# Unrepentant-Atheist/AC-3-ACM-Codec

Measured on AMD Instinct MI355X. Metric: AC-3 5.1@48kHz frames/sec/GPU (decode+encode); achieved HBM GB/s vs peak, higher is better.
Workload: dtype f32+i32

## Files before the change

### ac-3-acm-codec_amd/csrc/decode_mx.hip

```cpp
#include <stdlib.h>
#include "mant2.h"
#include "xform_core.h"
#include "ac3mi_internal.h"

namespace ac3mi {

constexpr int MX_PLANE = 256 + 16;
constexpr int MX_WAVE = 6 * EX_GROUP * 8;
constexpr int MX_RING = 6 * MX_PLANE * 4;
constexpr int MX_TILE = 3072;
static_assert(MX_RING + M2_LDS_WAVE <= MX_WAVE && MX_TILE + 256 * 6 * 2 <= MX_WAVE && 48 * 8 * 8 <= MX_TILE, "region layout");

struct MantxParams {
    MantParams m;
    const uint8_t *blksw;
    float *delay;
    const int32_t *slot;
    int delay_stride;
    float *pcm;
    int16_t *pcm16;
    int8_t wslot[6];
    const float2 *tw_long, *tw_short;
    const float *window;
    float bias;
};

struct MantxLDS {
    uint4 dsc[M2_NDESC];
    float qtab[760];
    float2 tw[2][128];
    float win[256];
    uint8_t cplbnd[6][20];
    uint32_t ready[6];
    alignas(16) uint8_t wave[6][MX_WAVE];
};

#ifndef MANTX_LB
#define MANTX_LB 3
#endif
#ifdef MX_STAMPS
__device__ unsigned long long g_mx_cycles[6][8];
#define MX_T0() unsigned long long mx_t = __builtin_readcyclecounter()
#define MX_LAP(id) do { const unsigned long long t_ = __builtin_readcyclecounter(); if (lane == 0) atomicAdd(&g_mx_cycles[blk][id], t_ - mx_t); mx_t = t_; } while (0)
#else
#define MX_T0() do { } while (0)
#define MX_LAP(id) do { } while (0)
#endif
template <bool S16>
__global__ __launch_bounds__(384, MANTX_LB) void mantx_kernel(const MantxParams Q)
{
    const MantParams &P = Q.m;
    __shared__ MantxLDS L;
    extern __shared__ uint32_t frw[];
    const int tid = threadIdx.x, lane = tid & 63;
    const int blk = __builtin_amdgcn_readfirstlane(tid >> 6);
    MX_T0();
    unsigned fidx;
    {
        const unsigned n = gridDim.x, q = n >> 3, r = n & 7u, x = blockIdx.x & 7u, i = blockIdx.x >> 3;
        fidx = (x < r ? x * (q + 1) : r * (q + 1) + (x - r) * q) + i;
    }
    const size_t unit = (size_t)fidx * 6 + blk;
    const uint4 *dq = reinterpret_cast<const uint4 *>(P.desc + unit);
    const uint4 w0v = dq[0], w1v = dq[1], w2v = dq[2], w3v = dq[3], w4v = dq[4];
    const uint32_t fposv = P.frame_pos[fidx];
    const int nw = (P.frame_bytes + 3) >> 2;
    {
        const uint32_t *s32 = reinterpret_cast<const uint32_t *>(P.frames + (size_t)fidx * P.frame_stride);
        for (int i = tid; i < nw + 6; i += 384) {
            uint32_t v = 0;
            if (i < nw) {
                v = s32[i];
                const int rem = P.frame_bytes - 4 * i;
                if (rem < 4) v &= (1u << (8 * rem)) - 1u;
                v = __builtin_bswap32(v);
            }
            frw[i] = v;
        }
        if (tid < M2_NDESC) L.dsc[tid] = mant_desc2((uint32_t)tid);
        for (int i = tid; i < 760; i += 384) L.qtab[i] = P.tab->qtab[i];
        if (tid < 128) L.tw[0][tid] = Q.tw_long[tid];
        else if (tid < 256) L.tw[1][tid - 128] = Q.tw_short[tid - 128];
        else L.win[tid - 256] = Q.window[tid - 256];
        if (tid < 128) L.win[128 + tid] = Q.window[128 + tid];
        if (tid < 6) L.ready[tid] = 0u;
    }
    uint8_t *const region = L.wave[blk];
    float *const planes = reinterpret_cast<float *>(region);
    const uint32_t flags = rfl(w0v.z);
    const bool failed = (flags & 1u) != 0u;
    MantBlk B;
    B.nf = P.nfchans; B.lfeon = P.lfeon; B.acmod = P.acmod; B.in_lfe = P.lfeon ? 1 : 0;
    B.chincpl = (int)((flags >> 8) & 31u); B.dithmask = (int)((flags >> 16) & 31u); B.rematflg = (int)((flags >> 24) & 15u);
    const uint64_t rve = (uint64_t)rfl(w2v.x) | ((uint64_t)rfl(w2v.y) << 32), rvb = (uint64_t)rfl(w2v.z) | ((uint64_t)rfl(w2v.w) << 32);
    const uint8_t *rowbase = P.rows + (size_t)fidx * 6 * ROWSET;
    auto fetch = [&](int slot) -> uint2 {
        const uint8_t *er = rowbase + (size_t)((rve >> (8 * slot)) & 7u) * ROWSET + slot * 512;
        const uint8_t *br = rowbase + (size_t)((rvb >> (8 * slot)) & 7u) * ROWSET + slot * 512 + 256;
        if (slot == 5) return lane < 7 ? make_uint2(br[lane], er[lane]) : make_uint2(1u, 0u);
        return make_uint2(reinterpret_cast<const uint32_t *>(br)[lane], reinterpret_cast<const uint32_t *>(er)[lane]);
    };
    const int slot0 = seg_slot(0, B.nf, B.chincpl, B.chincpl ? __builtin_ctz(B.chincpl) : 99);
    uint2 first = make_uint2(0u, 0u);
    if (!failed) first = fetch(slot0);
    __syncthreads();
    MX_LAP(0);

    if (failed) {
        for (int c = 0; c < P.n_in; c++)
            *reinterpret_cast<float4 *>(planes + c * MX_PLANE + 4 * lane) = make_float4(0.f, 0.f, 0.f, 0.f);
    } else {
        {
            const uint32_t a = rfl(w1v.x), b = rfl(w1v.y), c = rfl(w1v.z), d = rfl(w1v.w);
            B.cplstrtmant = (int)(c >> 16); B.cplendmant = (int)(d & 0xffffu);
            B.ends = (uint64_t)((a & 0xffu) | ((a >> 8) & 0xff00u) | ((b & 0xffu) << 16) | ((b << 8) & 0xff000000u)) | ((uint64_t)(c & 0xffu) << 32);
        }
        B.gainv = lane == 0 ? __uint_as_float(w3v.x) : lane == 1 ? __uint_as_float(w3v.y) : lane == 2 ? __uint_as_float(w3v.z)
                : lane == 3 ? __uint_as_float(w3v.w) : lane == 4 ? __uint_as_float(w4v.x) : __uint_as_float(w4v.y);
        if (B.chincpl && lane < 18) {
            const uint32_t below = rfl(w0v.w) & ((1u << lane) - 1u);
            L.cplbnd[blk][lane] = (uint8_t)(lane - __popc(below));
        }
        const uint32_t fpos = rfl(fposv);
        const bool lfsr_live = fpos != 0xffffffffu;
        const uint32_t i0 = lfsr_live ? (fpos + rfl(w0v.y)) % 65535u : 0u;
        const float *cc = P.cplco + unit * 90;
        mant_block2<MX_PLANE, true>(B, fetch, first, [&](int c, int bnd) { return cc[c * 18 + bnd]; }, L.cplbnd[blk], L.dsc, region + MX_RING, frw,
                              (uint32_t)nw + 2u, L.qtab, reinterpret_cast<const int16_t *>(P.lfsr_seq) + 1 + i0, lfsr_live, planes, rfl(w0v.x), lane);
    }
    __builtin_amdgcn_fence(__ATOMIC_RELEASE, "wavefront");
    __builtin_amdgcn_wave_barrier();
    __builtin_amdgcn_fence(__ATOMIC_ACQUIRE, "wavefront");

    MX_LAP(1);
    const int l8 = lane & 7, grp = lane >> 3;
    const bool own = grp < P.n_in;
    const int o = own ? grp : 0;
    const int fb = o - B.in_lfe;
    const bool sw = fb >= 0 && Q.blksw[unit * P.nfchans + fb] != 0;
    const size_t sidx = Q.slot ? (size_t)Q.slot[fidx] : (size_t)fidx;
    float *const dptr = Q.delay + sidx * Q.delay_stride + (size_t)o * 128;
    float2 dl[8];
    if (blk == 0) {
#pragma unroll
        for (int j = 0; j < 8; j++) {
            const int i = ((j & 1) ? 15 - l8 : l8) + 16 * (j >> 1);
            dl[j] = *reinterpret_cast<const float2 *>(dptr + 2 * i);
        }
    }
    FirstTail ft;
#pragma unroll
    for (int j = 0; j < 8; j++) ft.f0[j] = ft.f1[j] = ft.t0[j] = ft.t1[j] = 0.f;
    {
        const float *plane = planes + o * MX_PLANE;
        float xa[16], xb[16];
        if (!sw) {
            const float2 *p = reinterpret_cast<const float2 *>(plane) + l8;
            float2 v[16];
#pragma unroll
            for (int n = 0; n < 16; n++) v[n] = p[8 * n];
#pragma unroll
            for (int n = 0; n < 16; n++) {
                xa[n] = __builtin_fmaf(1.f, v[n].x, 0.f);
                xb[n] = __builtin_fmaf(1.f, mirror8(v[15 - n].y), 0.f);
            }
        } else {
            const int f = l8 >> 2, n2 = l8 & 3;
            const float *pa = plane + 4 * n2 + f;
            const float *pb = plane + 254 + f - 4 * n2;
#pragma unroll
            for (int n = 0; n < 16; n++) {
                xa[n] = __builtin_fmaf(1.f, pa[16 * n], 0.f);
                xb[n] = __builtin_fmaf(1.f, pb[-16 * n], 0.f);
            }
        }
        __builtin_amdgcn_fence(__ATOMIC_RELEASE, "wavefront");
        __builtin_amdgcn_wave_barrier();
        __builtin_amdgcn_fence(__ATOMIC_ACQUIRE, "wavefront");
        float2 *ex = reinterpret_cast<float2 *>(region) + o * EX_GROUP;
        const float2 *tw = &L.tw[sw ? 1 : 0][l8 * 16];
        cf r[16];
        imdct_first_half(xa, xb, tw, ex, l8, r);
        if (!sw) imdct_long_second_half(r, ft);
        else imdct_short_second_half(r, ft);
    }
    __builtin_amdgcn_fence(__ATOMIC_RELEASE, "wavefront");
    __builtin_amdgcn_wave_barrier();
    if (blk < 5 && lane < 48) {
        float2 *tl = reinterpret_cast<float2 *>(region);
#pragma unroll
        for (int j = 0; j < 8; j++) tl[j * 48 + lane] = make_float2(ft.t0[j], ft.t1[j]);
    }
    MX_LAP(2);
    if (blk == 0) asm volatile("s_waitcnt vmcnt(0)" ::: "memory");
    if (blk < 5) __hip_atomic_store(&L.ready[blk], 1u, __ATOMIC_RELEASE, __HIP_MEMORY_SCOPE_WORKGROUP);
    if (blk > 0) {
        for (int spin = 0; spin < (1 << 20) && __hip_atomic_load(&L.ready[blk - 1], __ATOMIC_ACQUIRE, __HIP_MEMORY_SCOPE_WORKGROUP) == 0u; spin++)
            __builtin_amdgcn_s_sleep(1);
        const float2 *tl = reinterpret_cast<const float2 *>(L.wave[blk - 1]);
        const int ls = lane < 48 ? lane : l8;
#pragma unroll
        for (int j = 0; j < 8; j++) dl[j] = tl[j * 48 + ls];
    }
    if (blk == 5) {
        for (int spin = 0; spin < (1 << 20) && __hip_atomic_load(&L.ready[0], __ATOMIC_ACQUIRE, __HIP_MEMORY_SCOPE_WORKGROUP) == 0u; spin++)
            __builtin_amdgcn_s_sleep(1);
    }
    if (blk == 5 && own) {
#pragma unroll
        for (int j = 0; j < 8; j++) {
            const int i = ((j & 1) ? 15 - l8 : l8) + 16 * (j >> 1);
            *reinterpret_cast<float2 *>(dptr + 2 * i) = make_float2(ft.t0[j], ft.t1[j]);
        }
    }

    MX_LAP(3);
    int16_t *tile = reinterpret_cast<int16_t *>(region + MX_TILE);
    int wsl = 0;
#pragma unroll
    for (int oo = 0; oo < 6; oo++) wsl = oo == o ? Q.wslot[oo] : wsl;
    float *oblk = S16 ? nullptr : Q.pcm + (unit * P.n_in + o) * 256;
#pragma unroll
    for (int j = 0; j < 8; j++) {
        const int i = ((j & 1) ? 15 - l8 : l8) + 16 * (j >> 1);
        const float2 wlo = *reinterpret_cast<const float2 *>(&L.win[2 * i]);
        const float2 whi = *reinterpret_cast<const float2 *>(&L.win[254 - 2 * i]);
        float2 lo, hi;
        window_pair(ft.f0[j], ft.f1[j], dl[j], wlo, whi, Q.bias, lo, hi);
        if (!S16 && own) {
            *reinterpret_cast<float2 *>(oblk + 2 * i) = lo;
            *reinterpret_cast<float2 *>(oblk + 254 - 2 * i) = hi;
        }
        if (S16 && own) {
            const int at = wsl + (int)__umul24((uint32_t)(2 * i), (uint32_t)P.n_in), top = wsl + (int)__umul24(254u, (uint32_t)P.n_in) - (at - wsl);
            tile[at] = to_s16(lo.x);
            tile[at + P.n_in] = to_s16(lo.y);
            tile[top] = to_s16(hi.x);
            tile[top + P.n_in] = to_s16(hi.y);
        }
    }
    if (S16) {
        __builtin_amdgcn_fence(__ATOMIC_RELEASE, "wavefront");
        __builtin_amdgcn_wave_barrier();
        __builtin_amdgcn_fence(__ATOMIC_ACQUIRE, "wavefront");
        const int upb = 32 * P.n_in;
        int16_t *dst = Q.pcm16 + unit * 256 * P.n_in;
#pragma unroll
        for (int it = 0; it < 3; it++) {
            const int u = it * 64 + lane;
            if (u < upb) *reinterpret_cast<uint4 *>(dst + u * 8) = *reinterpret_cast<const uint4 *>(tile + u * 8);
        }
    }
    MX_LAP(4);
}

hipError_t launch_mantx(const DeviceTables &tab, const DecodeLaunch &L, const MantParams &M, hipStream_t stream)
{
    const XformLaunch &X = *L.fuse;
    if (L.frames_per_stream != 1 || X.plan.n_in != X.plan.n_out || M.n_in > 6) return hipErrorInvalidValue;
    MantxParams Q;
    Q.m = M;
    Q.m.coef = nullptr;
    Q.blksw = L.blksw;
    Q.delay = X.delay;
    Q.slot = X.slot;
    Q.delay_stride = X.slot ? X.delay_stride : X.plan.n_out * 128;
    Q.pcm = X.pcm;
    Q.pcm16 = X.pcm16;
    Q.tw_long = tab.tw_long;
    Q.tw_short = tab.tw_short;
    Q.window = tab.window;
    Q.bias = X.bias;
    for (int o = 0; o < 6; o++) Q.wslot[o] = 0;
    static const int lds_pad = getenv("AC3MI_MANTX_LDS_PAD") ? atoi(getenv("AC3MI_MANTX_LDS_PAD")) : 0;
    const size_t dyn = (size_t)(((L.frame_bytes + 3) >> 2) + 6) * 4 + lds_pad;
    if (X.pcm16) {
        int map[6];
        if (s16_channel_map(X.s16_flags, map) != X.plan.n_out || ((uintptr_t)X.pcm16 & 15)) return hipErrorInvalidValue;
        for (int w = 0; w < X.plan.n_out; w++) Q.wslot[map[w]] = (int8_t)w;
        hipLaunchKernelGGL(mantx_kernel<true>, dim3(M.n_frames), dim3(384), dyn, stream, Q);
    } else {
        hipLaunchKernelGGL(mantx_kernel<false>, dim3(M.n_frames), dim3(384), dyn, stream, Q);
    }
    return hipGetLastError();
}

}

#ifdef MX_STAMPS
extern "C" __attribute__((visibility("default"))) int ac3mi_debug_mx_cycles(unsigned long long *out48, int reset)
{
    if (hipMemcpyFromSymbol(out48, HIP_SYMBOL(ac3mi::g_mx_cycles), sizeof(unsigned long long) * 48) != hipSuccess) return -1;
    if (reset) { unsigned long long z[48] = {0}; if (hipMemcpyToSymbol(HIP_SYMBOL(ac3mi::g_mx_cycles), z, sizeof z) != hipSuccess) return -1; }
    return 0;
}
#endif
```

### ac-3-acm-codec_amd/csrc/mant2.h

```cpp
#pragma once
#include "decode_common.h"

namespace ac3mi {

constexpr int M2_RING = 3 * 128;
constexpr int M2_LDS_WAVE = M2_RING + 256;
constexpr int M2_NDESC = 97;
constexpr int LFSR_EXT = 16384;

__host__ __device__ inline uint4 mant_desc2(uint32_t b)
{
    const uint32_t k1 = b >> 5, nbp = b >= 32 ? 0u : b == 1 ? 0u : b;
    const uint32_t inc = k1 == 1 ? 1u << 20 : k1 == 2 ? 1u << 10 : k1 == 3 ? 1u : 0u;
    const uint32_t obits = k1 == 1 ? 5u : k1 ? 7u : 0u, per = k1 == 3 ? 2u : k1 ? 3u : 0u, sh = 30u - 10u * k1;
    const uint32_t recip = k1 == 3 ? 1024u : k1 ? 683u : 0u;
    const uint32_t qbase = k1 == 1 ? 0u : k1 == 2 ? 96u : k1 == 3 ? 480u : nbp == 3 ? 736u : nbp == 4 ? 744u : 0u;
    const uint32_t coded = (k1 || nbp == 3 || nbp == 4) ? 1u : 0u, zero = b == 0 ? 1u : 0u;
    const uint32_t ring = k1 ? 128u * (k1 - 1u) : 0u;
    return make_uint4(inc, nbp | (obits << 8) | (per << 16) | (sh << 24), recip | (qbase << 16), ring | (zero << 16) | (coded << 24));
}

struct MantParams {
    const uint8_t *frames;
    const BlkDesc *desc;
    const uint8_t *rows;
    const float *cplco;
    const uint32_t *frame_pos;
    float *coef;
    const uint16_t *lfsr_seq;
    const DecTables *tab;
    unsigned n_frames;
    int frame_stride, frame_bytes;
    int acmod, lfeon, n_in, nfchans;
};

struct Seg2 {
    uint32_t bit;
    uint32_t phase;
    uint32_t draw;
};

template <int NB>
struct Bins2 {
    uint32_t raw[NB];
    uint32_t rs[NB];
    uint32_t dy[NB], dz[NB], dw[NB];
    uint32_t cd;
};

template <int NB>
__device__ __forceinline__ void seg2_first(uint32_t bytes4, const uint4 *dsc, uint8_t *ring, const uint32_t *frw, uint32_t frw_last,
                                           int mult, Seg2 &S, Bins2<NB> &R, int lane)
{
    uint32_t inc[NB], gl = 0;
#pragma unroll
    for (int j = 0; j < NB; j++) {
        const uint32_t b = (bytes4 >> (8 * j)) & 0xffu;
        const uint4 d = dsc[b];
        inc[j] = d.x; R.dy[j] = d.y; R.dz[j] = d.z; R.dw[j] = d.w;
        gl += d.x;
    }
    const uint32_t gin = wave_incl_scan_u32(gl);
    uint32_t run = gin - gl + S.phase;
    uint32_t nb[NB], nbsum = 0, ndsum = 0, slot[NB];
#pragma unroll
    for (int j = 0; j < NB; j++) {
        const uint32_t x = __builtin_amdgcn_ubfe(run, R.dy[j] >> 24, 10);
        run += inc[j];
        const uint32_t q = (x * (R.dz[j] & 0xffffu)) >> 11;
        const uint32_t mem = x - q * ((R.dy[j] >> 16) & 0xffu);
        const uint32_t ob = mem == 0u ? (R.dy[j] >> 8) & 0xffu : 0u;
        nb[j] = (R.dy[j] & 0xffu) + ob;
        nbsum += nb[j];
        ndsum += ((R.dw[j] >> 16) & 0xffu) * (uint32_t)mult;
        const uint32_t rslot = (R.dw[j] & 0xffffu) + (q & 127u);
        R.rs[j] = rslot | (mem << 16);
        slot[j] = ob != 0u ? rslot : (uint32_t)(M2_RING + 4 * lane);
    }
    const uint32_t bl = nbsum | (ndsum << 16);
    const uint32_t bin_ = wave_incl_scan_u32(bl);
    const uint32_t gtot = wave_last(gin), btot = wave_last(bin_);
    R.cd = S.draw + (bin_ >> 16) - ndsum;
    const uint32_t off = S.bit + (bin_ & 0xffffu) - nbsum;
    uint32_t wi = off >> 5;
    wi = wi < frw_last ? wi : frw_last;
    const uint32_t d0 = frw[wi], d1 = frw[wi + 1], d2 = frw[wi + 2];
    const uint32_t k = off & 31u;
    uint64_t win = ((((uint64_t)d0 << 32) | d1) << k) | (uint64_t)((d2 >> 1) >> (31u - k));
#pragma unroll
    for (int j = 0; j < NB; j++) {
        R.raw[j] = ((uint32_t)(win >> 32) >> 1) >> (31u - nb[j]);
        win <<= nb[j];
        ring[slot[j]] = (uint8_t)R.raw[j];
    }
    S.bit += btot & 0xffffu;
    S.draw += btot >> 16;
    {
        const uint32_t x3 = ((S.phase >> 20) & 1023u) + ((gtot >> 20) & 1023u), x5 = ((S.phase >> 10) & 1023u) + ((gtot >> 10) & 1023u),
                       x11 = (S.phase & 1023u) + (gtot & 1023u);
        const uint32_t q3 = (x3 * 683u) >> 11, q5 = (x5 * 683u) >> 11, q11 = x11 >> 1;
        S.phase = (((q3 & 127u) * 3u + (x3 - 3u * q3)) << 20) | (((q5 & 127u) * 3u + (x5 - 3u * q5)) << 10) | ((q11 & 127u) * 2u + (x11 & 1u));
    }
}

template <int NB>
__device__ __forceinline__ void seg2_values(const Bins2<NB> &R, const uint8_t *ring, const float *qtab, float *q)
{
    uint32_t code[NB];
#pragma unroll
    for (int j = 0; j < NB; j++) code[j] = ring[R.rs[j] & 0xffffu];
#pragma unroll
    for (int j = 0; j < NB; j++) { asm volatile("" : "+v"(code[j])); code[j] &= 0xffu; }
    float tv[NB];
#pragma unroll
    for (int j = 0; j < NB; j++) {
        const uint32_t per = (R.dy[j] >> 16) & 0xffu;
        const uint32_t sel = per ? code[j] * per + (R.rs[j] >> 16) : R.raw[j];
        tv[j] = qtab[(R.dw[j] >> 24) ? (R.dz[j] >> 16) + sel : 0u];
    }
#pragma unroll
    for (int j = 0; j < NB; j++) {
        const uint32_t nbp = R.dy[j] & 0xffu;
        const float pv = (float)(((int32_t)(R.raw[j] << ((32u - nbp) & 31u))) >> 16);
        q[j] = (R.dw[j] >> 24) ? tv[j] : pv;
    }
}

__device__ __forceinline__ float dither2(const int16_t *seq, uint32_t i) { return (float)((3 * (int)seq[i]) >> 2); }

template <int PS = 256, bool PK = false, class Fetch, class Cplco>
__device__ __forceinline__ void mant_block2(const MantBlk &B, Fetch fetch, uint2 first, Cplco cplco_of, const uint8_t *cplbnd, const uint4 *dsc, uint8_t *ring,
                                            const uint32_t *frw, uint32_t frw_last, const float *qtab, const int16_t *seq1, bool lfsr_live,
                                            float *cblk, uint32_t bitpos, int lane)
{
    const int nf = B.nf;
    const int ncpl_dith = __popc(B.chincpl & B.dithmask);
    const int em0 = PK ? (int)((uint32_t)B.ends & 0xffu) : B.endmant[0], em1 = PK ? (int)(((uint32_t)B.ends >> 8) & 0xffu) : B.endmant[1];
    const int remat_end = em0 < em1 ? em0 : em1;
    const bool remat_late = B.acmod == 2 && B.rematflg != 0 && B.chincpl != 0 && remat_end > B.cplstrtmant;
    const int cplfirst = B.chincpl ? __builtin_ctz(B.chincpl) : 99;
    const int nseg = nf + (B.chincpl ? 1 : 0) + (B.lfeon ? 1 : 0);
    Seg2 S;
    S.bit = bitpos;
    S.phase = 0;
    S.draw = 0;
    uint2 nxt = first;
    for (int k = 0; k < nseg; k++) {
        const int slot = seg_slot(k, nf, B.chincpl, cplfirst);
        const uint2 cur = nxt;
        if (k + 1 < nseg) nxt = fetch(seg_slot(k + 1, nf, B.chincpl, cplfirst));
        if (slot == 5) {
            Bins2<1> R;
            seg2_first<1>(lane < 7 ? cur.x & 0xffu : 1u, dsc, ring, frw, frw_last, 0, S, R, lane);
            __builtin_amdgcn_fence(__ATOMIC_RELEASE, "wavefront");
            __builtin_amdgcn_wave_barrier();
            __builtin_amdgcn_fence(__ATOMIC_ACQUIRE, "wavefront");
            float q;
            seg2_values<1>(R, ring, qtab, &q);
            const float lfe_gain = PK ? __builtin_bit_cast(float, __builtin_amdgcn_readlane(__builtin_bit_cast(int, B.gainv), 5)) : B.lfe_gain;
            const float v = q * (sf_of((int)(cur.y & 0xffu)) * lfe_gain);
            const float z = 0.f * (sf_of(0) * lfe_gain);
            if (lane < 8) cblk[lane] = lane < 7 ? v : z;
            if (lane >= 2) *reinterpret_cast<float4 *>(cblk + 4 * lane) = make_float4(z, z, z, z);
            continue;
        }
        int start = 0, end, draws;
        float g = 0.f;
        if (slot < 5) {
            if (PK) {
                end = (int)((uint32_t)(B.ends >> (8 * slot)) & 0xffu);
                g = __builtin_bit_cast(float, __builtin_amdgcn_readlane(__builtin_bit_cast(int, B.gainv), slot));
            } else {
                end = slot == 0 ? B.endmant[0] : slot == 1 ? B.endmant[1] : slot == 2 ? B.endmant[2] : slot == 3 ? B.endmant[3] : B.endmant[4];
                g = slot == 0 ? B.gain[0] : slot == 1 ? B.gain[1] : slot == 2 ? B.gain[2] : slot == 3 ? B.gain[3] : B.gain[4];
            }
            draws = (B.dithmask >> slot) & 1;
        } else {
            start = B.cplstrtmant;
            end = B.cplendmant;
            draws = ncpl_dith;
        }
        uint32_t bytes4;
        {
            int lo = start - 4 * lane, hi = end - 4 * lane;
            lo = lo < 0 ? 0 : lo > 4 ? 4 : lo;
            hi = hi < 0 ? 0 : hi > 4 ? 4 : hi;
            const uint32_t below_hi = (uint32_t)((1ull << (8 * hi)) - 1ull), below_lo = (uint32_t)((1ull << (8 * lo)) - 1ull);
            const uint32_t m = below_hi & ~below_lo;
            bytes4 = (cur.x & m) | (0x01010101u & ~m);
        }
        Bins2<4> R;
        seg2_first<4>(bytes4, dsc, ring, frw, frw_last, draws, S, R, lane);
        __builtin_amdgcn_fence(__ATOMIC_RELEASE, "wavefront");
        __builtin_amdgcn_wave_barrier();
        __builtin_amdgcn_fence(__ATOMIC_ACQUIRE, "wavefront");
        if (slot < 5) {
            float out[4], qv[4];
            seg2_values<4>(R, ring, qtab, qv);
            const bool dith = draws != 0 && lfsr_live;
            const uint32_t z0 = (R.dw[0] >> 16) & 0xffu, z1 = (R.dw[1] >> 16) & 0xffu, z2 = (R.dw[2] >> 16) & 0xffu, z3 = (R.dw[3] >> 16) & 0xffu;
            if (dith && __any((z0 | z1 | z2 | z3) != 0u)) {
                const int16_t *sp = seq1 + R.cd;
                const float d0 = dither2(sp, 0), d1 = dither2(sp, z0), d2 = dither2(sp, z0 + z1), d3 = dither2(sp, z0 + z1 + z2);
                qv[0] = z0 ? d0 : qv[0]; qv[1] = z1 ? d1 : qv[1]; qv[2] = z2 ? d2 : qv[2]; qv[3] = z3 ? d3 : qv[3];
            }
#pragma unroll
            for (int j = 0; j < 4; j++) {
                const int e = (int)((cur.y >> (8 * j)) & 0xffu);
                out[j] = qv[j] * (sf_of(e) * g);
            }
            float *plane = cblk + (slot + B.in_lfe) * PS;
            if (slot == 1 && B.acmod == 2 && B.rematflg != 0 && !remat_late) {
                float4 a4 = *reinterpret_cast<const float4 *>(plane - PS + 4 * lane);
                float a[4] = {a4.x, a4.y, a4.z, a4.w};
#pragma unroll
                for (int j = 0; j < 4; j++) {
                    const int bin = 4 * lane + j;
                    const int band = bin < 25 ? 0 : bin < 37 ? 1 : bin < 61 ? 2 : 3;
                    if (bin >= 13 && (bin < remat_end || (bin == 13 && remat_end <= 13)) && ((B.rematflg >> band) & 1)) {
                        const float x = a[j], v = out[j];
                        a[j] = x + v;
                        out[j] = x - v;
                    }
                }
                *reinterpret_cast<float4 *>(plane - PS + 4 * lane) = make_float4(a[0], a[1], a[2], a[3]);
            }
            if ((B.chincpl >> slot) & 1) {
#pragma unroll
                for (int j = 0; j < 4; j++) {
                    const int bin = 4 * lane + j;
                    if (bin < end || bin < B.cplstrtmant || bin >= B.cplendmant) plane[bin] = bin >= B.cplendmant ? 0.f : out[j];
                }
            } else {
                *reinterpret_cast<float4 *>(plane + 4 * lane) = make_float4(out[0], out[1], out[2], out[3]);
            }
        } else {
            uint32_t cd = R.cd;
            float qv[4];
            seg2_values<4>(R, ring, qtab, qv);
#pragma unroll
            for (int j = 0; j < 4; j++) {
                const int bin = 4 * lane + j;
                const bool in = bin >= start && bin < end;
                const bool zero = ((R.dw[j] >> 16) & 0xffu) != 0u;
                const int e = (int)((cur.y >> (8 * j)) & 0xffu);
                const float m = qv[j] * sf_of(e);
                const int bnd = cplbnd[in ? (bin - start) / 12 : 0];
                uint32_t cdc = cd;
                for (int c = 0; c < nf; c++) {
                    if (!((B.chincpl >> c) & 1)) continue;
                    const float gc = PK ? __builtin_bit_cast(float, __builtin_amdgcn_readlane(__builtin_bit_cast(int, B.gainv), c))
                                        : c == 0 ? B.gain[0] : c == 1 ? B.gain[1] : c == 2 ? B.gain[2] : c == 3 ? B.gain[3] : B.gain[4];
                    const float co = cplco_of(c, bnd) * gc;
                    float v = m * co;
                    if (zero) {
                        v = 0.f;
                        if ((B.dithmask >> c) & 1) { v = (sf_of(e) * co) * (lfsr_live ? dither2(seq1, cdc) : 0.f); cdc++; }
                    }
                    if (in) cblk[(c + B.in_lfe) * PS + bin] = v;
                }
                cd += zero ? (uint32_t)draws : 0u;
            }
        }
    }
    if (remat_late) {
        __builtin_amdgcn_fence(__ATOMIC_RELEASE, "wavefront");
        __builtin_amdgcn_wave_barrier();
        __builtin_amdgcn_fence(__ATOMIC_ACQUIRE, "wavefront");
        volatile float *p0 = cblk + (size_t)B.in_lfe * PS, *p1 = p0 + PS;
        for (int bin = 13 + lane; bin < remat_end; bin += 64) {
            const int band = bin < 25 ? 0 : bin < 37 ? 1 : bin < 61 ? 2 : 3;
            if ((B.rematflg >> band) & 1) {
                const float a = p0[bin], v = p1[bin];
                p0[bin] = a + v;
                p1[bin] = a - v;
            }
        }
    }
}

}
```

### ac-3-acm-codec_amd/csrc/xform_core.h

```cpp
#pragma once
#include <hip/hip_runtime.h>

namespace ac3mi {

struct cf { float re, im; };

__device__ __forceinline__ cf operator+(cf a, cf b) { return {a.re + b.re, a.im + b.im}; }
__device__ __forceinline__ cf operator-(cf a, cf b) { return {a.re - b.re, a.im - b.im}; }
__device__ __forceinline__ cf cmul(cf a, float cr, float ci)
{
    return {__builtin_fmaf(a.re, cr, -(a.im * ci)), __builtin_fmaf(a.re, ci, a.im * cr)};
}
__device__ __forceinline__ cf cmul(cf a, cf c) { return cmul(a, c.re, c.im); }

__device__ constexpr float C32_RE[16] = {
    1.000000000e+00f, 9.951847267e-01f, 9.807852804e-01f, 9.569403357e-01f, 9.238795325e-01f,
    8.819212643e-01f, 8.314696123e-01f, 7.730104534e-01f, 7.071067812e-01f, 6.343932842e-01f,
    5.555702330e-01f, 4.713967368e-01f, 3.826834324e-01f, 2.902846773e-01f, 1.950903220e-01f,
    9.801714033e-02f};
__device__ constexpr float C32_IM[16] = {
    -0.000000000e+00f, -9.801714033e-02f, -1.950903220e-01f, -2.902846773e-01f, -3.826834324e-01f,
    -4.713967368e-01f, -5.555702330e-01f, -6.343932842e-01f, -7.071067812e-01f, -7.730104534e-01f,
    -8.314696123e-01f, -8.819212643e-01f, -9.238795325e-01f, -9.569403357e-01f, -9.807852804e-01f,
    -9.951847267e-01f};

constexpr float K_C1 = 9.238795325e-01f;
constexpr float K_S1 = 3.826834324e-01f;
constexpr float K_R2 = 7.071067812e-01f;

__device__ __forceinline__ void dft4(cf &a, cf &b, cf &c, cf &d)
{
    cf s0 = a + c, s1 = a - c, s2 = b + d, s3 = b - d;
    a = s0 + s2;
    c = s0 - s2;
    b = {s1.re + s3.im, s1.im - s3.re};
    d = {s1.re - s3.im, s1.im + s3.re};
}

__device__ __forceinline__ void dft16(cf (&v)[16])
{
#pragma unroll
    for (int n2 = 0; n2 < 4; n2++) dft4(v[n2], v[4 + n2], v[8 + n2], v[12 + n2]);
    v[5] = cmul(v[5], K_C1, -K_S1);
    v[6] = {(v[6].re + v[6].im) * K_R2, (v[6].im - v[6].re) * K_R2};
    v[7] = cmul(v[7], K_S1, -K_C1);
    v[9] = {(v[9].re + v[9].im) * K_R2, (v[9].im - v[9].re) * K_R2};
    v[10] = {v[10].im, -v[10].re};
    v[11] = {(v[11].im - v[11].re) * K_R2, -(v[11].re + v[11].im) * K_R2};
    v[13] = cmul(v[13], K_S1, -K_C1);
    v[14] = {(v[14].im - v[14].re) * K_R2, -(v[14].re + v[14].im) * K_R2};
    v[15] = cmul(v[15], -K_C1, K_S1);
#pragma unroll
    for (int k1 = 0; k1 < 4; k1++) dft4(v[4 * k1], v[4 * k1 + 1], v[4 * k1 + 2], v[4 * k1 + 3]);
    cf t;
    t = v[1]; v[1] = v[4]; v[4] = t;
    t = v[2]; v[2] = v[8]; v[8] = t;
    t = v[3]; v[3] = v[12]; v[12] = t;
    t = v[6]; v[6] = v[9]; v[9] = t;
    t = v[7]; v[7] = v[13]; v[13] = t;
    t = v[11]; v[11] = v[14]; v[14] = t;
}

__device__ __forceinline__ void dft8(cf &a0, cf &a1, cf &a2, cf &a3, cf &a4, cf &a5, cf &a6, cf &a7)
{
    dft4(a0, a2, a4, a6);
    dft4(a1, a3, a5, a7);
    a3 = {(a3.re + a3.im) * K_R2, (a3.im - a3.re) * K_R2};
    a5 = {a5.im, -a5.re};
    a7 = {(a7.im - a7.re) * K_R2, -(a7.re + a7.im) * K_R2};
    cf x0 = a0 + a1, x4 = a0 - a1, x1 = a2 + a3, x5 = a2 - a3;
    cf x2 = a4 + a5, x6 = a4 - a5, x3 = a6 + a7, x7 = a6 - a7;
    a0 = x0; a1 = x1; a2 = x2; a3 = x3; a4 = x4; a5 = x5; a6 = x6; a7 = x7;
}

__device__ __forceinline__ float mirror8(float v)
{
    return __builtin_bit_cast(float, __builtin_amdgcn_update_dpp(0, __builtin_bit_cast(int, v), 0x141, 0xf, 0xf, false));
}

constexpr int EX_ROW = 18;
constexpr int EX_GROUP = 8 * EX_ROW + 8;
constexpr int EX_WAVE = 8 * EX_GROUP;

__device__ __forceinline__ void transpose_8x16_put(float2 *ex, int l8, const cf (&v)[16])
{
    float4 *row = reinterpret_cast<float4 *>(ex + l8 * EX_ROW);
#pragma unroll
    for (int j = 0; j < 8; j++) row[j] = make_float4(v[2 * j].re, v[2 * j].im, v[2 * j + 1].re, v[2 * j + 1].im);
    __builtin_amdgcn_fence(__ATOMIC_RELEASE, "wavefront");
    __builtin_amdgcn_wave_barrier();
    __builtin_amdgcn_fence(__ATOMIC_ACQUIRE, "wavefront");
}
__device__ __forceinline__ void transpose_8x16_get(const float2 *ex, int l8, cf (&r)[16])
{
#pragma unroll
    for (int l = 0; l < 8; l++) {
        float2 a = ex[l * EX_ROW + l8];
        float2 b = ex[l * EX_ROW + 15 - l8];
        r[l] = {a.x, a.y};
        r[8 + l] = {b.x, b.y};
    }
    __builtin_amdgcn_fence(__ATOMIC_RELEASE, "wavefront");
    __builtin_amdgcn_wave_barrier();
}
__device__ __forceinline__ void transpose_8x16(float2 *ex, int l8, const cf (&v)[16], cf (&r)[16])
{
    transpose_8x16_put(ex, l8, v);
    transpose_8x16_get(ex, l8, r);
}

__device__ constexpr float P16_RE[8] = {1.000000000e+00f, 9.807852804e-01f, 9.238795325e-01f, 8.314696123e-01f,
                                        7.071067812e-01f, 5.555702330e-01f, 3.826834324e-01f, 1.950903220e-01f};
__device__ constexpr float P16_IM[8] = {-0.000000000e+00f, -1.950903220e-01f, -3.826834324e-01f, -5.555702330e-01f,
                                        -7.071067812e-01f, -8.314696123e-01f, -9.238795325e-01f, -9.807852804e-01f};
__device__ constexpr float P8_RE[4] = {1.000000000e+00f, 9.238795325e-01f, 7.071067812e-01f, 3.826834324e-01f};
__device__ constexpr float P8_IM[4] = {-0.000000000e+00f, -3.826834324e-01f, -7.071067812e-01f, -9.238795325e-01f};

struct FirstTail {
    float f0[8], f1[8], t0[8], t1[8];
};

__device__ __forceinline__ cf tw_at(const cf (&tw)[16], int k) { return tw[k]; }
__device__ __forceinline__ cf tw_at(const float2 *tw, int k) { float2 t = tw[k]; return {t.x, t.y}; }

template <typename TW>
__device__ __forceinline__ void imdct_first_half_put(const float (&xa)[16], const float (&xb)[16], const TW &tw, float2 *ex, int l8)
{
    cf v[16];
#pragma unroll
    for (int n = 0; n < 16; n++) v[n] = cmul(cf{xa[n], xb[n]}, C32_RE[n], C32_IM[n]);
    dft16(v);
#pragma unroll
    for (int k = 0; k < 16; k++) v[k] = cmul(v[k], tw_at(tw, k));
    transpose_8x16_put(ex, l8, v);
}
template <typename TW>
__device__ __forceinline__ void imdct_first_half(const float (&xa)[16], const float (&xb)[16], const TW &tw,
                                                 float2 *ex, int l8, cf (&r)[16])
{
    imdct_first_half_put(xa, xb, tw, ex, l8);
    transpose_8x16_get(ex, l8, r);
}

__device__ __forceinline__ void window_pair(float f0, float f1, float2 d, float2 wlo, float2 whi, float bias, float2 &lo, float2 &hi)
{
    lo.x = __builtin_fmaf(f0, wlo.x, __builtin_fmaf(d.x, whi.y, bias));
    lo.y = __builtin_fmaf(f1, wlo.y, __builtin_fmaf(d.y, whi.x, bias));
    hi.x = __builtin_fmaf(-f1, whi.x, __builtin_fmaf(d.y, wlo.y, bias));
    hi.y = __builtin_fmaf(-f0, whi.y, __builtin_fmaf(d.x, wlo.x, bias));
}

__device__ __forceinline__ int16_t to_s16(float v)
{
    int i = (int)(__float_as_uint(v) - 0x43c00000u);
    i = i > 32767 ? 32767 : i < -32768 ? -32768 : i;
    return (int16_t)i;
}

__device__ __forceinline__ void imdct_long_second_half(cf (&r)[16], FirstTail &ft);
__device__ __forceinline__ void imdct_short_second_half(cf (&r)[16], FirstTail &ft);

template <typename TW>
__device__ __forceinline__ void imdct_long(const float (&xa)[16], const float (&xb)[16], const TW &tw,
                                           float2 *ex, int l8, FirstTail &ft)
{
    cf r[16];
    imdct_first_half(xa, xb, tw, ex, l8, r);
    imdct_long_second_half(r, ft);
}

__device__ __forceinline__ void imdct_long_second_half(cf (&r)[16], FirstTail &ft)
{
    dft8(r[0], r[1], r[2], r[3], r[4], r[5], r[6], r[7]);
    dft8(r[8], r[9], r[10], r[11], r[12], r[13], r[14], r[15]);
#pragma unroll
    for (int k = 1; k < 8; k++) {
        r[k] = cmul(r[k], P16_RE[k], P16_IM[k]);
        r[8 + k] = cmul(r[8 + k], P16_RE[k], P16_IM[k]);
    }
#pragma unroll
    for (int k = 0; k < 4; k++) {
        ft.f0[2 * k] += -r[k].re;
        ft.t0[2 * k] += -r[k].im;
        ft.f1[2 * k] += r[15 - k].re;
        ft.t1[2 * k] += -r[15 - k].im;
        ft.f0[2 * k + 1] += -r[8 + k].re;
        ft.t0[2 * k + 1] += -r[8 + k].im;
        ft.f1[2 * k + 1] += r[7 - k].re;
        ft.t1[2 * k + 1] += -r[7 - k].im;
    }
}

template <typename TW>
__device__ __forceinline__ void imdct_short(const float (&xa)[16], const float (&xb)[16], const TW &tw,
                                            float2 *ex, int l8, FirstTail &ft)
{
    cf r[16];
    imdct_first_half(xa, xb, tw, ex, l8, r);
    imdct_short_second_half(r, ft);
}

__device__ __forceinline__ void imdct_short_second_half(cf (&r)[16], FirstTail &ft)
{
    dft4(r[0], r[1], r[2], r[3]);
    dft4(r[4], r[5], r[6], r[7]);
    dft4(r[8], r[9], r[10], r[11]);
    dft4(r[12], r[13], r[14], r[15]);
#pragma unroll
    for (int k = 1; k < 4; k++) {
        r[k] = cmul(r[k], P8_RE[k], P8_IM[k]);
        r[4 + k] = cmul(r[4 + k], P8_RE[k], P8_IM[k]);
        r[8 + k] = cmul(r[8 + k], P8_RE[k], P8_IM[k]);
        r[12 + k] = cmul(r[12 + k], P8_RE[k], P8_IM[k]);
    }
#pragma unroll
    for (int k = 0; k < 4; k++) {
        ft.f0[2 * k] += -r[k].re;
        ft.t0[2 * k] += -r[4 + k].im;
        ft.f1[2 * k] += r[11 - k].im;
        ft.t1[2 * k] += r[15 - k].re;
        ft.f0[2 * k + 1] += -r[8 + k].re;
        ft.t0[2 * k + 1] += -r[12 + k].im;
        ft.f1[2 * k + 1] += r[3 - k].im;
        ft.t1[2 * k + 1] += r[7 - k].re;
    }
}

}
```

Baseline: 8.789 million.

## Shrink mantx LDS footprint to fit more workgroups per CU

Shrinks per-wave LDS regions to 1 KB per channel group and moves the LFE plane into a compact 16-float slot. The 760-entry float quant table becomes byte indices into a 48-entry level table. Twiddle and window tables are now read from global memory instead of being staged in LDS, and the IMDCT transpose uses XOR-swizzled addressing. The delay-line load moves after the transform behind an extra ready flag, and the 16-bit variant gets higher launch bounds. The aim is more workgroups per CU and less prologue staging, at the cost of global/cache reads for tables and an extra indirection per dequantized value.

```diff
diff --git a/ac-3-acm-codec_amd/csrc/decode_mx.hip b/ac-3-acm-codec_amd/csrc/decode_mx.hip
--- a/ac-3-acm-codec_amd/csrc/decode_mx.hip
+++ b/ac-3-acm-codec_amd/csrc/decode_mx.hip
@@ -6,10 +6,35 @@
 namespace ac3mi {
 
 constexpr int MX_PLANE = 256 + 16;
-constexpr int MX_WAVE = 6 * EX_GROUP * 8;
-constexpr int MX_RING = 6 * MX_PLANE * 4;
+constexpr int MX_LFE = 3 * MX_PLANE + 256;
+constexpr int MX_WAVE = 6 * 1024;
+constexpr int MX_RING = (4 * MX_PLANE + 256) * 4;
+constexpr int MX_CPLB = MX_RING + M2_LDS_WAVE;
 constexpr int MX_TILE = 3072;
-static_assert(MX_RING + M2_LDS_WAVE <= MX_WAVE && MX_TILE + 256 * 6 * 2 <= MX_WAVE && 48 * 8 * 8 <= MX_TILE, "region layout");
+static_assert(MX_LFE + 16 <= 4 * MX_PLANE && MX_CPLB + 20 <= MX_WAVE && MX_TILE + 256 * 6 * 2 <= MX_WAVE && 48 * 8 * 8 <= MX_TILE,
+              "region layout");
+
+__device__ __forceinline__ void mx_transpose_put(uint8_t *W, uint32_t wb, const cf (&v)[16])
+{
+#pragma unroll
+    for (int j = 0; j < 8; j++)
+        *reinterpret_cast<float4 *>(W + (wb ^ (uint32_t)(16 * j))) = make_float4(v[2 * j].re, v[2 * j].im, v[2 * j + 1].re, v[2 * j + 1].im);
+    __builtin_amdgcn_fence(__ATOMIC_RELEASE, "wavefront");
+    __builtin_amdgcn_wave_barrier();
+    __builtin_amdgcn_fence(__ATOMIC_ACQUIRE, "wavefront");
+}
+__device__ __forceinline__ void mx_transpose_get(const uint8_t *W, uint32_t ra, uint32_t rb, cf (&r)[16])
+{
+#pragma unroll
+    for (int l = 0; l < 8; l++) {
+        const float2 a = *reinterpret_cast<const float2 *>(W + (ra ^ (uint32_t)(144 * l)));
+        const float2 b = *reinterpret_cast<const float2 *>(W + (rb ^ (uint32_t)(144 * l)));
+        r[l] = {a.x, a.y};
+        r[8 + l] = {b.x, b.y};
+    }
+    __builtin_amdgcn_fence(__ATOMIC_RELEASE, "wavefront");
+    __builtin_amdgcn_wave_barrier();
+}
 
 struct MantxParams {
     MantParams m;
@@ -26,17 +51,19 @@
 };
 
 struct MantxLDS {
+    alignas(16) uint8_t wave[6][MX_WAVE];
     uint4 dsc[M2_NDESC];
-    float qtab[760];
-    float2 tw[2][128];
-    float win[256];
-    uint8_t cplbnd[6][20];
+    float qlev[48];
     uint32_t ready[6];
-    alignas(16) uint8_t wave[6][MX_WAVE];
+    uint8_t qidx[760];
 };
+static_assert(sizeof(MantxLDS) + (384 + 6) * 4 <= 40960, "mantx_kernel: four workgroups per CU at 384 kb/s");
 
 #ifndef MANTX_LB
 #define MANTX_LB 3
+#endif
+#ifndef MANTX_LB16
+#define MANTX_LB16 6
 #endif
 #ifdef MX_STAMPS
 __device__ unsigned long long g_mx_cycles[6][8];
@@ -47,7 +74,7 @@
 #define MX_LAP(id) do { } while (0)
 #endif
 template <bool S16>
-__global__ __launch_bounds__(384, MANTX_LB) void mantx_kernel(const MantxParams Q)
+__global__ __launch_bounds__(384, S16 ? MANTX_LB16 : MANTX_LB) void mantx_kernel(const MantxParams Q)
 {
     const MantParams &P = Q.m;
     __shared__ MantxLDS L;
@@ -78,15 +105,13 @@
             frw[i] = v;
         }
         if (tid < M2_NDESC) L.dsc[tid] = mant_desc2((uint32_t)tid);
-        for (int i = tid; i < 760; i += 384) L.qtab[i] = P.tab->qtab[i];
-        if (tid < 128) L.tw[0][tid] = Q.tw_long[tid];
-        else if (tid < 256) L.tw[1][tid - 128] = Q.tw_short[tid - 128];
-        else L.win[tid - 256] = Q.window[tid - 256];
-        if (tid < 128) L.win[128 + tid] = Q.window[128 + tid];
+        for (int i = tid; i < 760; i += 384) L.qidx[i] = (uint8_t)qtab_level((uint32_t)i);
+        if (tid < 48) L.qlev[tid] = P.tab->qlev[tid];
         if (tid < 6) L.ready[tid] = 0u;
     }
     uint8_t *const region = L.wave[blk];
     float *const planes = reinterpret_cast<float *>(region);
+    uint8_t *const cplbnd = region + MX_CPLB;
     const uint32_t flags = rfl(w0v.z);
     const bool failed = (flags & 1u) != 0u;
     MantBlk B;
@@ -107,9 +132,12 @@
     MX_LAP(0);
 
     if (failed) {
-        for (int c = 0; c < P.n_in; c++)
+#pragma unroll
+        for (int c = 0; c < 5; c++)
             *reinterpret_cast<float4 *>(planes + c * MX_PLANE + 4 * lane) = make_float4(0.f, 0.f, 0.f, 0.f);
+        if (lane < 4) *reinterpret_cast<float4 *>(planes + MX_LFE + 4 * lane) = make_float4(0.f, 0.f, 0.f, 0.f);
     } else {
+        if (B.in_lfe && B.nf < 5) *reinterpret_cast<float4 *>(planes + 4 * MX_PLANE + 4 * lane) = make_float4(0.f, 0.f, 0.f, 0.f);
         {
             const uint32_t a = rfl(w1v.x), b = rfl(w1v.y), c = rfl(w1v.z), d = rfl(w1v.w);
             B.cplstrtmant = (int)(c >> 16); B.cplendmant = (int)(d & 0xffffu);
@@ -119,14 +147,15 @@
                 : lane == 3 ? __uint_as_float(w3v.w) : lane == 4 ? __uint_as_float(w4v.x) : __uint_as_float(w4v.y);
         if (B.chincpl && lane < 18) {
             const uint32_t below = rfl(w0v.w) & ((1u << lane) - 1u);
-            L.cplbnd[blk][lane] = (uint8_t)(lane - __popc(below));
+            cplbnd[lane] = (uint8_t)(lane - __popc(below));
         }
         const uint32_t fpos = rfl(fposv);
         const bool lfsr_live = fpos != 0xffffffffu;
         const uint32_t i0 = lfsr_live ? (fpos + rfl(w0v.y)) % 65535u : 0u;
         const float *cc = P.cplco + unit * 90;
-        mant_block2<MX_PLANE, true>(B, fetch, first, [&](int c, int bnd) { return cc[c * 18 + bnd]; }, L.cplbnd[blk], L.dsc, region + MX_RING, frw,
-                              (uint32_t)nw + 2u, L.qtab, reinterpret_cast<const int16_t *>(P.lfsr_seq) + 1 + i0, lfsr_live, planes, rfl(w0v.x), lane);
+        mant_block2<MX_PLANE, true, true>(B, fetch, first, [&](int c, int bnd) { return cc[c * 18 + bnd]; }, cplbnd, L.dsc, region + MX_RING, frw,
+                                          (uint32_t)nw + 2u, QTab2{L.qidx, L.qlev}, reinterpret_cast<const int16_t *>(P.lfsr_seq) + 1 + i0, lfsr_live,
+                                          planes - B.in_lfe * MX_PLANE, rfl(w0v.x), lane, planes + MX_LFE);
     }
     __builtin_amdgcn_fence(__ATOMIC_RELEASE, "wavefront");
     __builtin_amdgcn_wave_barrier();
@@ -135,34 +164,28 @@
     MX_LAP(1);
     const int l8 = lane & 7, grp = lane >> 3;
     const bool own = grp < P.n_in;
-    const int o = own ? grp : 0;
+    const int o = own ? grp : (grp & 3) < P.n_in ? (grp & 3) : 0;
     const int fb = o - B.in_lfe;
     const bool sw = fb >= 0 && Q.blksw[unit * P.nfchans + fb] != 0;
     const size_t sidx = Q.slot ? (size_t)Q.slot[fidx] : (size_t)fidx;
     float *const dptr = Q.delay + sidx * Q.delay_stride + (size_t)o * 128;
     float2 dl[8];
-    if (blk == 0) {
-#pragma unroll
-        for (int j = 0; j < 8; j++) {
-            const int i = ((j & 1) ? 15 - l8 : l8) + 16 * (j >> 1);
-            dl[j] = *reinterpret_cast<const float2 *>(dptr + 2 * i);
-        }
-    }
     FirstTail ft;
 #pragma unroll
     for (int j = 0; j < 8; j++) ft.f0[j] = ft.f1[j] = ft.t0[j] = ft.t1[j] = 0.f;
     {
-        const float *plane = planes + o * MX_PLANE;
+        const float *plane = fb >= 0 ? planes + fb * MX_PLANE : planes + MX_LFE;
         float xa[16], xb[16];
         if (!sw) {
             const float2 *p = reinterpret_cast<const float2 *>(plane) + l8;
             float2 v[16];
 #pragma unroll
             for (int n = 0; n < 16; n++) v[n] = p[8 * n];
+            const float mz = fb >= 0 ? 1.f : 0.f;
 #pragma unroll
             for (int n = 0; n < 16; n++) {
-                xa[n] = __builtin_fmaf(1.f, v[n].x, 0.f);
-                xb[n] = __builtin_fmaf(1.f, mirror8(v[15 - n].y), 0.f);
+                xa[n] = __builtin_fmaf(n == 0 ? 1.f : mz, v[n].x, 0.f);
+                xb[n] = __builtin_fmaf(n == 15 ? 1.f : mz, mirror8(v[15 - n].y), 0.f);
             }
         } else {
             const int f = l8 >> 2, n2 = l8 & 3;
@@ -177,10 +200,17 @@
         __builtin_amdgcn_fence(__ATOMIC_RELEASE, "wavefront");
         __builtin_amdgcn_wave_barrier();
         __builtin_amdgcn_fence(__ATOMIC_ACQUIRE, "wavefront");
-        float2 *ex = reinterpret_cast<float2 *>(region) + o * EX_GROUP;
-        const float2 *tw = &L.tw[sw ? 1 : 0][l8 * 16];
+        const uint32_t gb = (uint32_t)blk * MX_WAVE + (uint32_t)o * 1024u, h4 = (uint32_t)(o & 2) << 1, l8u = (uint32_t)l8;
+        const uint32_t wb = gb + ((l8u ^ (uint32_t)(o & 1)) << 7) + ((l8u ^ h4) << 4);
+        const uint32_t ra = gb + ((uint32_t)(o & 1) << 7) + (((l8u >> 1) ^ h4) << 4) + ((l8u & 1u) << 3);
+        const float2 *tw = (sw ? Q.tw_short : Q.tw_long) + l8 * 16;
         cf r[16];
-        imdct_first_half(xa, xb, tw, ex, l8, r);
+        {
+            cf v[16];
+            imdct_first_half_v(xa, xb, tw, v);
+            mx_transpose_put(reinterpret_cast<uint8_t *>(L.wave), wb, v);
+        }
+        mx_transpose_get(reinterpret_cast<const uint8_t *>(L.wave), ra, ra ^ 0x78u, r);
         if (!sw) imdct_long_second_half(r, ft);
         else imdct_short_second_half(r, ft);
     }
@@ -192,8 +222,16 @@
         for (int j = 0; j < 8; j++) tl[j * 48 + lane] = make_float2(ft.t0[j], ft.t1[j]);
     }
     MX_LAP(2);
-    if (blk == 0) asm volatile("s_waitcnt vmcnt(0)" ::: "memory");
     if (blk < 5) __hip_atomic_store(&L.ready[blk], 1u, __ATOMIC_RELEASE, __HIP_MEMORY_SCOPE_WORKGROUP);
+    if (blk == 0) {
+#pragma unroll
+        for (int j = 0; j < 8; j++) {
+            const int i = ((j & 1) ? 15 - l8 : l8) + 16 * (j >> 1);
+            dl[j] = *reinterpret_cast<const float2 *>(dptr + 2 * i);
+        }
+        asm volatile("s_waitcnt vmcnt(0)" ::: "memory");
+        __hip_atomic_store(&L.ready[5], 1u, __ATOMIC_RELEASE, __HIP_MEMORY_SCOPE_WORKGROUP);
+    }
     if (blk > 0) {
         for (int spin = 0; spin < (1 << 20) && __hip_atomic_load(&L.ready[blk - 1], __ATOMIC_ACQUIRE, __HIP_MEMORY_SCOPE_WORKGROUP) == 0u; spin++)
             __builtin_amdgcn_s_sleep(1);
@@ -203,7 +241,7 @@
         for (int j = 0; j < 8; j++) dl[j] = tl[j * 48 + ls];
     }
     if (blk == 5) {
-        for (int spin = 0; spin < (1 << 20) && __hip_atomic_load(&L.ready[0], __ATOMIC_ACQUIRE, __HIP_MEMORY_SCOPE_WORKGROUP) == 0u; spin++)
+        for (int spin = 0; spin < (1 << 20) && __hip_atomic_load(&L.ready[5], __ATOMIC_ACQUIRE, __HIP_MEMORY_SCOPE_WORKGROUP) == 0u; spin++)
             __builtin_amdgcn_s_sleep(1);
     }
     if (blk == 5 && own) {
@@ -223,8 +261,8 @@
 #pragma unroll
     for (int j = 0; j < 8; j++) {
         const int i = ((j & 1) ? 15 - l8 : l8) + 16 * (j >> 1);
-        const float2 wlo = *reinterpret_cast<const float2 *>(&L.win[2 * i]);
-        const float2 whi = *reinterpret_cast<const float2 *>(&L.win[254 - 2 * i]);
+        const float2 wlo = *reinterpret_cast<const float2 *>(Q.window + 2 * i);
+        const float2 whi = *reinterpret_cast<const float2 *>(Q.window + 254 - 2 * i);
         float2 lo, hi;
         window_pair(ft.f0[j], ft.f1[j], dl[j], wlo, whi, Q.bias, lo, hi);
         if (!S16 && own) {
diff --git a/ac-3-acm-codec_amd/csrc/mant2.h b/ac-3-acm-codec_amd/csrc/mant2.h
--- a/ac-3-acm-codec_amd/csrc/mant2.h
+++ b/ac-3-acm-codec_amd/csrc/mant2.h
@@ -103,8 +103,24 @@
     }
 }
 
-template <int NB>
-__device__ __forceinline__ void seg2_values(const Bins2<NB> &R, const uint8_t *ring, const float *qtab, float *q)
+struct QTab2 {
+    const uint8_t *idx;
+    const float *lev;
+};
+__device__ __forceinline__ float qtab_at(const float *t, uint32_t i) { return t[i]; }
+__device__ __forceinline__ float qtab_at(const QTab2 &t, uint32_t i) { return t.lev[t.idx[i]]; }
+
+__host__ __device__ inline uint32_t qtab_level(uint32_t i)
+{
+    if (i < 96) { const uint32_t c = i / 3, m = i % 3; return c >= 27 ? 43u : m == 0 ? c / 9 : m == 1 ? (c / 3) % 3 : c % 3; }
+    if (i < 480) { const uint32_t c = (i - 96) / 3, m = (i - 96) % 3; return c >= 125 ? 43u : 3u + (m == 0 ? c / 25 : m == 1 ? (c / 5) % 5 : c % 5); }
+    if (i < 736) { const uint32_t c = (i - 480) / 2, m = (i - 480) % 2; return c >= 121 ? 43u : 16u + (m == 0 ? c / 11 : c % 11); }
+    if (i < 744) return i - 736 < 7 ? 8u + (i - 736) : 43u;
+    return i - 744 < 15 ? 27u + (i - 744) : 43u;
+}
+
+template <int NB, class QT>
+__device__ __forceinline__ void seg2_values(const Bins2<NB> &R, const uint8_t *ring, const QT &qtab, float *q)
 {
     uint32_t code[NB];
 #pragma unroll
@@ -116,7 +132,7 @@
     for (int j = 0; j < NB; j++) {
         const uint32_t per = (R.dy[j] >> 16) & 0xffu;
         const uint32_t sel = per ? code[j] * per + (R.rs[j] >> 16) : R.raw[j];
-        tv[j] = qtab[(R.dw[j] >> 24) ? (R.dz[j] >> 16) + sel : 0u];
+        tv[j] = qtab_at(qtab, (R.dw[j] >> 24) ? (R.dz[j] >> 16) + sel : 0u);
     }
 #pragma unroll
     for (int j = 0; j < NB; j++) {
@@ -128,10 +144,10 @@
 
 __device__ __forceinline__ float dither2(const int16_t *seq, uint32_t i) { return (float)((3 * (int)seq[i]) >> 2); }
 
-template <int PS = 256, bool PK = false, class Fetch, class Cplco>
+template <int PS = 256, bool PK = false, bool LFE16 = false, class Fetch, class Cplco, class QT>
 __device__ __forceinline__ void mant_block2(const MantBlk &B, Fetch fetch, uint2 first, Cplco cplco_of, const uint8_t *cplbnd, const uint4 *dsc, uint8_t *ring,
-                                            const uint32_t *frw, uint32_t frw_last, const float *qtab, const int16_t *seq1, bool lfsr_live,
-                                            float *cblk, uint32_t bitpos, int lane)
+                                            const uint32_t *frw, uint32_t frw_last, const QT &qtab, const int16_t *seq1, bool lfsr_live,
+                                            float *cblk, uint32_t bitpos, int lane, float *lfe = nullptr)
 {
     const int nf = B.nf;
     const int ncpl_dith = __popc(B.chincpl & B.dithmask);
@@ -160,8 +176,12 @@
             const float lfe_gain = PK ? __builtin_bit_cast(float, __builtin_amdgcn_readlane(__builtin_bit_cast(int, B.gainv), 5)) : B.lfe_gain;
             const float v = q * (sf_of((int)(cur.y & 0xffu)) * lfe_gain);
             const float z = 0.f * (sf_of(0) * lfe_gain);
-            if (lane < 8) cblk[lane] = lane < 7 ? v : z;
-            if (lane >= 2) *reinterpret_cast<float4 *>(cblk + 4 * lane) = make_float4(z, z, z, z);
+            if (LFE16) {
+                if (lane < 16) lfe[lane] = lane < 7 ? v : z;
+            } else {
+                if (lane < 8) cblk[lane] = lane < 7 ? v : z;
+                if (lane >= 2) *reinterpret_cast<float4 *>(cblk + 4 * lane) = make_float4(z, z, z, z);
+            }
             continue;
         }
         int start = 0, end, draws;
diff --git a/ac-3-acm-codec_amd/csrc/xform_core.h b/ac-3-acm-codec_amd/csrc/xform_core.h
--- a/ac-3-acm-codec_amd/csrc/xform_core.h
+++ b/ac-3-acm-codec_amd/csrc/xform_core.h
@@ -124,14 +124,19 @@
 __device__ __forceinline__ cf tw_at(const float2 *tw, int k) { float2 t = tw[k]; return {t.x, t.y}; }
 
 template <typename TW>
-__device__ __forceinline__ void imdct_first_half_put(const float (&xa)[16], const float (&xb)[16], const TW &tw, float2 *ex, int l8)
-{
-    cf v[16];
+__device__ __forceinline__ void imdct_first_half_v(const float (&xa)[16], const float (&xb)[16], const TW &tw, cf (&v)[16])
+{
 #pragma unroll
     for (int n = 0; n < 16; n++) v[n] = cmul(cf{xa[n], xb[n]}, C32_RE[n], C32_IM[n]);
     dft16(v);
 #pragma unroll
     for (int k = 0; k < 16; k++) v[k] = cmul(v[k], tw_at(tw, k));
+}
+template <typename TW>
+__device__ __forceinline__ void imdct_first_half_put(const float (&xa)[16], const float (&xb)[16], const TW &tw, float2 *ex, int l8)
+{
+    cf v[16];
+    imdct_first_half_v(xa, xb, tw, v);
     transpose_8x16_put(ex, l8, v);
 }
 template <typename TW>
```

After: 8.897 million, median of 6. 1.01x the previous value.
